# CityU-AIM-Group/HTD

Hardware: AMD Instinct MI355X
Metric: images/sec (1333x800) HTD-R50 train step (higher is better)
Workload: dtype f32; 1 GPU; HTD ResNet-50 FPN fp32 train step fwd+bwd+SGD, batch 4/GPU @ 1333x800 (padded 1344x800), random-init weights, 2000 RPN proposals/img, 512 RoIs/img/stage; global_batch=4, parallelism=dp1, stage2_positives=168, proposals=random-init RPN (few positives: the regression branch is nearly idle)

## Files before the change

### htd_amd/csrc/conv_x3.hip

```cpp
#include <algorithm>
#include <mutex>
#include <type_traits>
#include <unordered_map>

#include <stdlib.h>

#include "common.h"

namespace {

using f32x16 = __attribute__((ext_vector_type(16))) float;
using bf16x8 = __attribute__((ext_vector_type(8))) __bf16;
using bf16x2 = __attribute__((ext_vector_type(2))) __bf16;
using f32x2 = __attribute__((ext_vector_type(2))) float;
using f32x4 = __attribute__((ext_vector_type(4))) float;

using f16x8 = __attribute__((ext_vector_type(8))) _Float16;
using f16x2 = __attribute__((ext_vector_type(2))) _Float16;

constexpr int XK = 16;
constexpr int NCH = 6;

struct H2Scale { float s, inv; };
__device__ __forceinline__ H2Scale h2_scale(const float *amax)
// ... 1227 lines not shown
    int lo = 0, hi = n - 1;
    const int64_t b = blockIdx.x;
    while (lo < hi) {
        const int mid = (lo + hi + 1) >> 1;
        if (descs[mid].row0 <= b) lo = mid;
        else hi = mid - 1;
    }
    const PlanesDescH d = descs[lo];
    const int tr = d.transposed & 1;
    const int N = tr ? d.Ci : d.Co, K = tr ? d.Co : d.Ci;
    const int Np = ((N + 127) / 128) * 128;
    float *scales = reinterpret_cast<float *>(d.out + planes_vec(d.taps, K, Np));
    const int groups = Np / 64, r = (int)(b - d.row0);
    x3h_rowmax_part(d.w, scales + 2 * Np, d.Co, d.taps, d.Ci, Np, tr, (r % groups) * 64, r / groups, red);
}

__global__ __launch_bounds__(256) void x3h_planes_many_kernel(const PlanesDescH *__restrict__ descs, int n)
{
    int lo = 0, hi = n - 1;
    const int64_t b = blockIdx.x;
    while (lo < hi) {
        const int mid = (lo + hi + 1) >> 1;
        if (descs[mid].block0 <= b) lo = mid;
        else hi = mid - 1;
    }
    const PlanesDescH d = descs[lo];
    const int tr = d.transposed & 1;
    const int N = tr ? d.Ci : d.Co, K = tr ? d.Co : d.Ci;
    const int Np = ((N + 127) / 128) * 128;
    const int64_t total = (int64_t)d.taps * (K / XK) * Np;
    const int64_t e = (b - d.block0) * 256 + threadIdx.x;
    float *scales = reinterpret_cast<float *>(d.out + planes_vec(d.taps, K, Np));
    if (e < total) x3h_planes_element(d.w, d.out, scales, d.Co, d.taps, d.Ci, Np, tr, e);
}

__global__ __launch_bounds__(256) void absmax_kernel(const float *__restrict__ x, int64_t n, unsigned *__restrict__ out)
{
    const int64_t n4 = n >> 2;
    float mx = 0.f;
    unsigned nan = 0u;
    const float4 *x4 = reinterpret_cast<const float4 *>(x);
    const int64_t stride = (int64_t)gridDim.x * 256;
    int64_t i = (int64_t)blockIdx.x * 256 + threadIdx.x;
    for (; i + 3 * stride < n4; i += 4 * stride) {
        const float4 a = x4[i], b = x4[i + stride], c = x4[i + 2 * stride], d = x4[i + 3 * stride];
        const float m0 = fmaxf(fmaxf(fabsf(a.x), fabsf(a.y)), fmaxf(fabsf(a.z), fabsf(a.w)));
        const float m1 = fmaxf(fmaxf(fabsf(b.x), fabsf(b.y)), fmaxf(fabsf(b.z), fabsf(b.w)));
        const float m2 = fmaxf(fmaxf(fabsf(c.x), fabsf(c.y)), fmaxf(fabsf(c.z), fabsf(c.w)));
        const float m3 = fmaxf(fmaxf(fabsf(d.x), fabsf(d.y)), fmaxf(fabsf(d.z), fabsf(d.w)));
        mx = fmaxf(fmaxf(mx, fmaxf(m0, m1)), fmaxf(m2, m3));
        const float t = (a.x - a.x) + (a.y - a.y) + (a.z - a.z) + (a.w - a.w) + (b.x - b.x) + (b.y - b.y) + (b.z - b.z) + (b.w - b.w) +
                        (c.x - c.x) + (c.y - c.y) + (c.z - c.z) + (c.w - c.w) + (d.x - d.x) + (d.y - d.y) + (d.z - d.z) + (d.w - d.w);
        if (t != t) {
            nan |= (a.x != a.x) | (a.y != a.y) | (a.z != a.z) | (a.w != a.w) | (b.x != b.x) | (b.y != b.y) | (b.z != b.z) | (b.w != b.w) |
                   (c.x != c.x) | (c.y != c.y) | (c.z != c.z) | (c.w != c.w) | (d.x != d.x) | (d.y != d.y) | (d.z != d.z) | (d.w != d.w);
        }
    }
    for (; i < n4; i += stride) {
        const float4 v = x4[i];
        mx = fmaxf(fmaxf(mx, fmaxf(fabsf(v.x), fabsf(v.y))), fmaxf(fabsf(v.z), fabsf(v.w)));
        nan |= (v.x != v.x) | (v.y != v.y) | (v.z != v.z) | (v.w != v.w);
    }
    if (blockIdx.x == 0 && threadIdx.x < (n & 3)) {
        const float t = x[(n4 << 2) + threadIdx.x];
        mx = fmaxf(mx, fabsf(t));
        nan |= t != t;
// ... 378 lines not shown
                       Ci, Np, transposed);
    return htd::check_launch("x3h_planes");
}

extern "C" int htd_conv2d_x3h_planes_many(const void *desc, int n, int64_t total_blocks, int64_t total_rows, void *stream)
{
    static_assert(sizeof(PlanesDescH) == 48, "PlanesDescH layout is part of the ABI");
    HTD_REQUIRE(desc && n > 0 && total_blocks > 0 && total_blocks < (1ll << 31) && total_rows > 0 && total_rows < (1ll << 31),
                "x3h_planes_many: bad arguments");
    hipLaunchKernelGGL(x3h_rowscale_many_kernel, dim3((unsigned)total_rows), dim3(256), 0, (hipStream_t)stream,
                       (const PlanesDescH *)desc, n);
    hipLaunchKernelGGL(x3h_planes_many_kernel, dim3((unsigned)total_blocks), dim3(256), 0, (hipStream_t)stream,
                       (const PlanesDescH *)desc, n);
    return htd::check_launch("x3h_planes_many");
}

extern "C" int htd_absmax(const float *x, int64_t n, float *amax, void *stream)
{
    HTD_REQUIRE(x && amax && n > 0 && ((uintptr_t)x & 15) == 0, "absmax: bad arguments");
    const unsigned blocks = (unsigned)std::min<int64_t>(htd::ceil_div(n >> 2, (int64_t)256 * 8) + 1, 2048);
    hipLaunchKernelGGL(absmax_kernel, dim3(blocks), dim3(256), 0, (hipStream_t)stream, x, n, (unsigned *)amax);
    return htd::check_launch("absmax");
}

extern "C" int htd_conv2d_x3_planes_many(const void *desc, int n, int64_t total_blocks, void *stream)
{
    static_assert(sizeof(PlanesDesc) == 40, "PlanesDesc layout is part of the ABI");
    HTD_REQUIRE(desc && n > 0 && total_blocks > 0 && total_blocks < (1ll << 31), "x3_planes_many: bad arguments");
    hipLaunchKernelGGL(x3_planes_many_kernel, dim3((unsigned)total_blocks), dim3(256), 0, (hipStream_t)stream,
                       (const PlanesDesc *)desc, n);
    return htd::check_launch("x3_planes_many");
}

extern "C" int64_t htd_conv2d_x3p_workspace_bytes(int64_t M, int Co, int Ci, int kh, int kw)
{
    int64_t need = 0;
    for (int cfg = 0; cfg < 4; ++cfg) need = std::max(need, plan_x3p(cfg, M, Co, (Ci / XK) * kh, kw, true).partial_floats * 4);
    return need;
}

extern "C" int64_t htd_act_planes_rows(int64_t M) { return M > 0 ? act_rows(M) : 0; }

extern "C" int64_t htd_act_planes_bytes(int64_t M, int C)
{
    if (M <= 0 || C <= 0 || C % XK != 0) return 0;
    return (int64_t)(C / XK) * NCH * act_rows(M) * 16;
}

extern "C" int htd_act_planes(const float *x, void *planes, int64_t M, int C, void *stream)
{
    HTD_REQUIRE(x && planes && M > 0 && C > 0 && C % XK == 0, "act_planes: bad arguments (C %% 16)");
    const unsigned blocks = (unsigned)std::min<int64_t>(htd::ceil_div(M * (C >> 3), (int64_t)256), 65536);
    hipLaunchKernelGGL(act_planes_kernel, dim3(blocks), dim3(256), 0, (hipStream_t)stream, x, (uint4 *)planes, M, C, act_rows(M));
    return htd::check_launch("act_planes");
}

extern "C" int htd_conv2d_fwd_x3q(const float *x, const void *xplanes, const void *wplanes, const float *bias,
                                  const float *residual, int res_h, int res_w, float *y, void *yplanes, float *amax_out, int B, int H,
                                  int W, int Ci, int Co, int kh, int kw, int stride, int pad, int relu, void *workspace, void *stream)
{
    HTD_REQUIRE((x || xplanes) && wplanes && y && B > 0 && H > 0 && W > 0, "conv2d_fwd_x3q: bad arguments");
    HTD_REQUIRE(x3p_shape_ok(Ci, Co, kh, kw, stride, pad, 1), "conv2d_fwd_x3q: unsupported layer Ci=%d Co=%d k=%dx%d s=%d p=%d", Ci,
                Co, kh, kw, stride, pad);
    HTD_REQUIRE(!xplanes || (kh == 1 && stride == 1), "conv2d_fwd_x3q: input planes serve 1x1 / stride-1 layers only");
    HTD_REQUIRE(!yplanes || Co % XK == 0, "conv2d_fwd_x3q: output planes need Co %% 16 == 0 (Co=%d)", Co);
    HTD_REQUIRE((res_h > 0) == (res_w > 0) && res_h >= 0 && (res_h == 0 || ((Co & 3) == 0 && residual)),
// ... 214 lines not shown
```

### htd_amd/dense.py

```python
import os

import torch
from torch.autograd import Function
from torch.autograd.function import once_differentiable
from torch.multiprocessing.reductions import StorageWeakRef as _StorageWeakRef

from . import capi

CL = torch.channels_last
_P = capi.ptr
_S = capi.current_stream_ptr


def _out_hw(H, W, kh, kw, stride, pad, dil):
    return ((H + 2 * pad - (dil * (kh - 1) + 1)) // stride + 1, (W + 2 * pad - (dil * (kw - 1) + 1)) // stride + 1)


def _need_gpu(t, name):
    if not t.is_cuda:
        raise NotImplementedError(f'{name}: only GPU tensors are supported (libhtd_amd.so has no CPU path)')


def _splitk_ws(M, Co, Cred, kh, kw, device):
    nbytes = capi.lib().htd_conv2d_workspace_bytes(M, Co, Cred, kh, kw)
    return torch.empty(nbytes // 4, device=device, dtype=torch.float32) if nbytes > 0 else None


_GRAD_SINK = {}


def register_grad_sinks(params, views, used):
    import weakref
    keys = []
    for p, v in zip(params, views):
        _GRAD_SINK[p.data_ptr()] = (v, weakref.ref(p), used)
        keys.append(p.data_ptr())
    used.clear()
    return keys


# ... 112 lines not shown
    return s


def mark_side_consumed(t):
    _SIDE_CONSUMED.add(t.data_ptr())


_FLIPPED = {}


def offer_flipped(weight, wT):
    _FLIPPED[weight.data_ptr()] = wT


def take_flipped(weight):
    return _FLIPPED.pop(weight.data_ptr(), None)


_STEP_FLIPS = {}


_M = None


def _flip_key(w):
    global _M
    if _M is None:
        from . import mmcv_ops
        _M = mmcv_ops
    return (w.data_ptr(), w._version, tuple(w.shape), _M.PARAM_EPOCH)


def new_step():
    _STEP_FLIPS.clear()
    _STEP_PLANES.clear()
    _AMAX_POOL.clear()
    _AMAX_BY_PTR.clear()
    _drop_temp_sinks()


_AMAX_POOL = {}
_AMAX_SLOTS = 1024
H2_1X1 = os.environ.get('HTD_H2_1X1', '1') != '0'
H2_CHECK = os.environ.get('HTD_H2_CHECK', '0') == '1'
H2_ABSMAX_MIN_WORK = int(os.environ.get('HTD_H2_ABSMAX_MIN_WORK', '2304'))
H2_ABSMAX_MIN_ELEMS = int(os.environ.get('HTD_H2_ABSMAX_MIN_ELEMS', str(1 << 20)))


def _x3h_ok(Cred, Cout, kh, kw, stride, padding, dilation, dtype):
    return dtype == torch.float32 and (kh == 3 or H2_1X1) and \
        bool(capi.lib().htd_conv2d_x3h_supported(Cred, Cout, kh, kw, stride, padding, dilation))


def _amax_slot(device):
    ent = _AMAX_POOL.get(device.index)
    if ent is None or ent[1] >= _AMAX_SLOTS:
        ent = [torch.zeros(_AMAX_SLOTS, device=device, dtype=torch.float32), 0]
        _AMAX_POOL[device.index] = ent
    slot = ent[0][ent[1]:ent[1] + 1]
    ent[1] += 1
    return slot


def absmax(x):
    slot = _amax_slot(x.device)
    capi.call('htd_absmax', _P(x), x.numel(), _P(slot), _S(), work=('byte', 4.0 * x.numel()))
# ... 73 lines not shown
    if a is None or a[1] != t.data_ptr() or a[2] != t.numel() or a[3] != t._version:
        return None
    if H2_CHECK:
        fresh = absmax(t)
        if not torch.equal(fresh, a[0]) and not (torch.isnan(fresh).item() and torch.isnan(a[0]).item()):
            raise RuntimeError(f'stale carried maximum: {float(a[0])} against {float(fresh)} on a tensor of shape {tuple(t.shape)}')
    return a[0]


_STEP_PLANES = {}


def _planes_key(w, transposed):
    return _flip_key(w) + (bool(transposed), )


_ALSO_WANTED = set()


def _planes_h2(w, transposed):
    Co, Ci, kh, kw = w.shape
    cred, cout = (Co, Ci) if transposed else (Ci, Co)
    return kh == kw and _x3h_ok(cred, cout, kh, kw, 1, kh // 2, 1, w.dtype)


def x3_planes(weight, transposed, h2=None):
    if h2 is None:
        h2 = _planes_h2(weight, transposed)
    key = _planes_key(weight, transposed) + (bool(h2), )
    hit = _STEP_PLANES.get(key)
    if hit is not None:
        return hit[1]
    _ALSO_WANTED.add((tuple(weight.shape), bool(transposed), bool(h2)))
    Co, Ci, kh, kw = weight.shape
    nbytes = capi.lib().htd_conv2d_x3_planes_bytes(Co, kh, kw, Ci, int(transposed))
    planes = torch.empty(nbytes // 4, device=weight.device, dtype=torch.int32)
    capi.call('htd_conv2d_x3h_planes' if h2 else 'htd_conv2d_x3_planes', _P(weight), _P(planes), Co, kh, kw, Ci, int(transposed), _S())
    _STEP_PLANES[key] = (weight, planes)
    return planes


def _planes_wanted(w, transposed):
    Co, Ci, kh, kw = w.shape
    cred, cout = (Co, Ci) if transposed else (Ci, Co)
    return w.is_cuda and w.dtype == torch.float32 and kh == kw and kh in (1, 3) and w.is_contiguous(memory_format=CL) and \
        bool(capi.lib().htd_conv2d_x3p_supported(cred, cout, kh, kw, 1, kh // 2, 1))


def planes_many(items):
    import numpy as np
    todo, seen = [], set()
    for w, tr in items:
        w4 = w if w.dim() == 4 else w.view(w.size(0), w.size(1), 1, 1)
        if not _planes_wanted(w4, tr):
            continue
        h2 = _planes_h2(w4, tr)
        for v in ((h2, ) if (tuple(w4.shape), bool(tr), not h2) not in _ALSO_WANTED else (h2, not h2)):
            key = _planes_key(w4, tr) + (v, )
            if key not in _STEP_PLANES and key not in seen:
                seen.add(key)
                todo.append((key, w4, tr))
    if not todo:
        return
    L = capi.lib()
    dev = todo[0][1].device
    for h2 in (False, True):
# ... 4 lines not shown
        flat = torch.empty(sum(sizes), device=dev, dtype=torch.int32)
        desc = np.zeros((len(part), 6 if h2 else 5), dtype=np.int64)
        off = block0 = row0 = 0
        for i, ((key, w, tr), n32) in enumerate(zip(part, sizes)):
            out = flat[off:off + n32]
            off += n32
            Co, Ci, taps = w.size(0), w.size(1), w.size(2) * w.size(3)
            N = Ci if tr else Co
            Np = (N + 127) // 128 * 128
            desc[i, 0], desc[i, 1] = w.data_ptr(), out.data_ptr()
            desc[i, 2] = Co | (taps << 32)
            desc[i, 3] = Ci | (int(tr) << 32)
            desc[i, 4] = block0
            K = Co if tr else Ci
            nch = (taps * K + 1023) // 1024
            if h2:
                desc[i, 5] = row0
                row0 += Np // 64 * nch
            block0 += ((n32 - (2 + nch) * Np) // 4 // 6 + 255) // 256
            _STEP_PLANES[key] = (w, out)
        table = capi.upload_table(desc, dev)
        if h2:
            capi.call('htd_conv2d_x3h_planes_many', _P(table), len(part), block0, row0, _S())
        else:
            capi.call('htd_conv2d_x3_planes_many', _P(table), len(part), block0, _S())


def _x3p_ok(Cred, Cout, kh, kw, stride, padding, dilation, dtype):
    return dtype == torch.float32 and bool(capi.lib().htd_conv2d_x3p_supported(Cred, Cout, kh, kw, stride, padding, dilation))


def flip_many(weights):
    import numpy as np
    ws, pl = [], []
    for w in weights:
        w4 = w if w.dim() == 4 else w.view(w.size(0), w.size(1), 1, 1)
        pl += [(w4, False), (w4, True)]
        if w4.is_cuda and w4.dtype == torch.float32 and w4.size(0) % 8 == 0 and w4.is_contiguous(memory_format=CL) and \
                _flip_key(w4) not in _STEP_FLIPS and not _planes_wanted(w4, True):
            ws.append(w4)
    planes_many(pl)
    if not ws:
        return
    dev = ws[0].device
    flat = torch.empty(sum(w.numel() for w in ws), device=dev, dtype=torch.float32)
    desc = np.zeros((len(ws), 10), dtype=np.int64)
    off = tile0 = 0
    for i, w in enumerate(ws):
        Co, Ci, taps = w.size(0), w.size(1), w.size(2) * w.size(3)
        wT = flat[off:off + w.numel()]
        off += w.numel()
        desc[i, 0], desc[i, 7] = w.data_ptr(), wT.data_ptr()
        desc[i, 8] = Co | (Ci << 32)
        desc[i, 9] = taps | (tile0 << 32)
        tile0 += taps * ((Co + 31) // 32) * ((Ci + 31) // 32)
        _STEP_FLIPS[_flip_key(w)] = (w, wT)
    table = capi.upload_table(desc, dev)
    capi.call('htd_bn_fold_many_fwd', _P(table), len(ws), tile0, 0.0, _S())


def join_side_stream():
    if _SIDE:
        cur = torch.cuda.current_stream()
        s = _SIDE.get(cur.device.index)
        if s is not None:
            cur.wait_stream(s)
# ... 1069 lines not shown
```

### htd_amd/detector/bricks.py

```python
import torch
import torch.nn as nn
import torch.nn.functional as F

from .. import mmcv_ops as M
from ..registry import CONV_LAYERS

CL = torch.channels_last


def dense_conv2d(x, weight, bias=None, stride=1, padding=0, dilation=1, relu=False, residual=None, residual_up=False,
                 chain=False):
    from .. import dense
    if x.dtype == torch.bfloat16:
        y = dense.conv2d_bf16_autograd(x, weight, bias, stride, padding, dilation, relu, residual, residual_up)
        return (y, x) if chain else y
    return dense.conv2d(x, weight, bias, stride, padding, dilation, relu, residual, residual_up, chain)


@CONV_LAYERS.register_module('Conv')
@CONV_LAYERS.register_module('Conv2d')
class Conv2d(nn.Conv2d):

    def __init__(self, *args, **kwargs):
        super().__init__(*args, **kwargs)
# ... 72 lines not shown
        w, gamma, mean, var = ctx.saved_tensors
        Co = w.size(0)
        K = w.numel() // Co
        gwf = gwf.contiguous(memory_format=CL)
        gbf = gbf.contiguous()
        from .. import dense

        def launch():
            (gw, s1), (gg, s2), (gb, s3) = dense.grad_out2(w), dense.grad_out2(gamma), dense.grad_out2(ctx.beta_ref)
            capi.call('htd_bn_fold_bwd', capi.ptr(w), capi.ptr(gamma), capi.ptr(mean), capi.ptr(var), ctx.eps,
                      capi.ptr(gwf), capi.ptr(gbf), capi.ptr(gw), capi.ptr(gg), capi.ptr(gb), Co, K,
                      capi.current_stream_ptr())
            return (gw, gg, gb), s1 and s2 and s3
        if not dense.OVERLAP_WGRAD or (capi.profiling() and not dense._OVERLAP_IN_PROFILE):
            return launch()[0] + (None, None, None)
        main, side = torch.cuda.current_stream(), dense.side_stream(gwf.device)
        side.wait_stream(main)
        gwf.record_stream(side)
        gbf.record_stream(side)
        with torch.cuda.stream(side):
            outs, all_sinks = launch()
        if not all_sinks:
            for t in outs:
                t.record_stream(main)
            main.wait_stream(side)
        return outs + (None, None, None)


class _BNFoldMany(torch.autograd.Function):

    @staticmethod
    def forward(ctx, eps, want_flips, want_planes, *tensors):
        import numpy as np
        from .. import capi, dense
        n = len(tensors) // 5
        dev = tensors[0].device
        ws = [tensors[5 * i].contiguous(memory_format=CL) for i in range(n)]
        sizes = [(w.size(0), w.size(1), w.size(2) * w.size(3)) for w in ws]
        total = sum(2 * w.numel() + w.size(0) for w in ws) if want_flips else sum(w.numel() + w.size(0) for w in ws)
        flat = torch.empty(total, device=dev, dtype=torch.float32)
        desc = np.zeros((n, 10), dtype=np.int64)
        outs, flips, off, tile0 = [], [], 0, 0
        for i, (w, (Co, Ci, taps)) in enumerate(zip(ws, sizes)):
            wf = flat[off:off + w.numel()].view(Co, w.size(2), w.size(3), Ci).permute(0, 3, 1, 2)
            off += w.numel()
            bf = flat[off:off + Co]
            off += Co
            wT = None
            if want_flips:
                wT = flat[off:off + w.numel()]
                off += w.numel()
            g, b, m, v = tensors[5 * i + 1:5 * i + 5]
            desc[i, :8] = (w.data_ptr(), g.data_ptr(), b.data_ptr(), m.data_ptr(), v.data_ptr(), wf.data_ptr(), bf.data_ptr(),
                           wT.data_ptr() if wT is not None else 0)
            desc[i, 8] = Co | (Ci << 32)
            desc[i, 9] = taps | (tile0 << 32)
            tile0 += taps * ((Co + 31) // 32) * ((Ci + 31) // 32)
            outs += [wf, bf]
            flips.append(wT)
        table = capi.upload_table(desc, dev)
        capi.call('htd_bn_fold_many_fwd', capi.ptr(table), n, tile0, float(eps), capi.current_stream_ptr())
        if want_planes:
            dense.planes_many([(wf, False) for wf in outs[0::2]] + ([(wf, True) for wf in outs[0::2]] if want_flips else []))
        for wf, wT in zip(outs[0::2], flips):
            dense.mark_side_consumed(wf)
            if wT is not None:
                dense.offer_flipped(wf, wT)
        ctx.save_for_backward(*[t for i in range(n) for t in (ws[i], tensors[5 * i + 1], tensors[5 * i + 3], tensors[5 * i + 4])])
        ctx.beta_refs = [tensors[5 * i + 2] for i in range(n)]
        ctx.eps, ctx.n = float(eps), n
        return tuple(outs)

    @staticmethod
    @torch.autograd.function.once_differentiable
    def backward(ctx, *grads):
        import numpy as np
        from .. import capi, dense
        n, saved = ctx.n, ctx.saved_tensors
        dev = saved[0].device

        def launch():
            desc = np.zeros((n, 11), dtype=np.int64)
            outs, row0, all_sinks, keep = [], 0, True, []
            for i in range(n):
                w, gamma, mean, var = saved[4 * i:4 * i + 4]
                Co, K = w.size(0), w.numel() // w.size(0)
                gwf, gbf = grads[2 * i], grads[2 * i + 1]
                gwf = torch.zeros_like(w, memory_format=CL) if gwf is None else gwf.contiguous(memory_format=CL)
                gbf = torch.zeros(Co, device=dev) if gbf is None else gbf.contiguous()
                keep += [gwf, gbf]
                (gw, s1), (gg, s2), (gb, s3) = dense.grad_out2(w), dense.grad_out2(gamma), dense.grad_out2(ctx.beta_refs[i])
                all_sinks = all_sinks and s1 and s2 and s3
                desc[i, :9] = (w.data_ptr(), gamma.data_ptr(), mean.data_ptr(), var.data_ptr(), gwf.data_ptr(), gbf.data_ptr(),
                               gw.data_ptr(), gg.data_ptr(), gb.data_ptr())
                desc[i, 9] = Co | (K << 32)
                desc[i, 10] = row0
                row0 += Co
                outs.append((gw, gg, gb))
            table = capi.upload_table(desc, dev)
            capi.call('htd_bn_fold_many_bwd', capi.ptr(table), n, row0, ctx.eps, capi.current_stream_ptr())
            return outs, all_sinks, keep
        if not dense.OVERLAP_WGRAD or (capi.profiling() and not dense._OVERLAP_IN_PROFILE):
            outs = launch()[0]
        else:
            main, side = torch.cuda.current_stream(), dense.side_stream(dev)
            side.wait_stream(main)
            with torch.cuda.stream(side):
                outs, all_sinks, keep = launch()
            for t in keep:
                t.record_stream(side)
            if not all_sinks:
                for trio in outs:
                    for t in trio:
                        t.record_stream(main)
                main.wait_stream(side)
        res = [None, None, None]
        for gw, gg, gb in outs:
            res += [gw, gg, gb, None, None]
        return tuple(res)


def frozen_bn_fold_many(pairs, want_flips=True, want_planes=True):
    ok = torch.is_grad_enabled() and all(w.is_cuda and w.dtype == torch.float32 and (w.numel() // w.size(0)) % 4 == 0 and
                                          not bn.training for w, bn in pairs)
    if not ok or len({bn.eps for _, bn in pairs}) != 1:
        out = []
        for w, bn in pairs:
            out += frozen_bn_fold(w, bn)
        return out
    args = []
    for w, bn in pairs:
        args += [w, bn.weight, bn.bias, bn.running_mean, bn.running_var]
    return list(_BNFoldMany.apply(pairs[0][1].eps, bool(want_flips), bool(want_planes), *args))


def frozen_bn_fold(conv_weight, bn):
    if conv_weight.is_cuda and (conv_weight.numel() // conv_weight.size(0)) % 4 == 0:
        if torch.is_grad_enabled():
            return _BNFold.apply(conv_weight, bn.weight, bn.bias, bn.running_mean, bn.running_var, bn.eps)
        key = (M.PARAM_EPOCH, conv_weight.data_ptr(), conv_weight._version, bn.weight._version, bn.bias._version,
               bn.running_mean._version, bn.running_var._version)
        cached = bn.__dict__.get('_htd_fold_cache')
        if cached is None or cached[0] != key:
            cached = (key, _BNFold.apply(conv_weight, bn.weight, bn.bias, bn.running_mean, bn.running_var, bn.eps))
            bn.__dict__['_htd_fold_cache'] = cached
        return cached[1]
    s = bn.weight * torch.rsqrt(bn.running_var + bn.eps)
    return conv_weight * s.view(-1, 1, 1, 1), bn.bias - bn.running_mean * s


def kaiming_init(module, a=0, mode='fan_out', nonlinearity='relu', bias=0, distribution='normal'):
    if distribution == 'uniform':
        nn.init.kaiming_uniform_(module.weight, a=a, mode=mode, nonlinearity=nonlinearity)
    else:
        nn.init.kaiming_normal_(module.weight, a=a, mode=mode, nonlinearity=nonlinearity)
    if getattr(module, 'bias', None) is not None:
        nn.init.constant_(module.bias, bias)


def xavier_init(module, gain=1, bias=0, distribution='normal'):
    if distribution == 'uniform' and gain == 1 and hasattr(module, 'tile_shape'):
        module.xavier_uniform_()
# ... 67 lines not shown
```

### htd_amd/detector/resnet.py

```python
import math
import os

import torch
import torch.nn as nn
from torch.nn.modules.batchnorm import _BatchNorm

from .. import mmcv_ops as M
from ..dense import ResStageBf16Function, ResStageFunction
from ..registry import BACKBONES
from .bricks import build_conv_layer, build_norm_layer, constant_init, frozen_bn_fold, frozen_bn_fold_many, kaiming_init

CL = torch.channels_last
FUSE_BF16_STAGE = os.environ.get('HTD_BF16_STAGE', '1') != '0'


def conv_bn(conv, bn, x, relu=False, residual=None):
    if bn.training:
        y = bn(conv(x))
        if residual is not None:
            y = y + residual
        return torch.relu(y) if relu else y
    w, b = frozen_bn_fold(conv.weight, bn)
    return conv(x, relu=relu, residual=residual, weight=w, bias=b)

# ... 72 lines not shown

class ResLayer(nn.Sequential):
    def __init__(self, block, inplanes, planes, num_blocks, stride=1, avg_down=False, conv_cfg=None,
                 norm_cfg=dict(type='BN'), downsample_first=True, **kwargs):
        assert not avg_down and downsample_first, 'ResNetV1d / hourglass variants are outside the HTD path'
        self.block = block
        downsample = None
        if stride != 1 or inplanes != planes * block.expansion:
            downsample = nn.Sequential(
                build_conv_layer(conv_cfg, inplanes, planes * block.expansion, kernel_size=1, stride=stride, bias=False),
                build_norm_layer(norm_cfg, planes * block.expansion)[1])
        layers = [block(inplanes=inplanes, planes=planes, stride=stride, downsample=downsample, conv_cfg=conv_cfg,
                        norm_cfg=norm_cfg, **kwargs)]
        inplanes = planes * block.expansion
        for _ in range(1, num_blocks):
            layers.append(block(inplanes=inplanes, planes=planes, stride=1, conv_cfg=conv_cfg, norm_cfg=norm_cfg,
                                **kwargs))
        super().__init__(*layers)

    def _fusable(self):
        for blk in self:
            if not isinstance(blk, Bottleneck) or blk.with_dcn or blk.style != 'pytorch' or blk.groups != 1:
                return False
            bns = [blk.norm1, blk.norm2, blk.norm3] + ([blk.downsample[1]] if blk.downsample is not None else [])
            if any(bn.training or not isinstance(bn, nn.BatchNorm2d) for bn in bns):
                return False
        return True

    def forward(self, x, chain=False):
        if not x.is_cuda or x.dtype not in (torch.float32, torch.bfloat16) or not self._fusable() or \
                (x.dtype == torch.bfloat16 and not FUSE_BF16_STAGE):
            y = super().forward(x)
            return (y, x) if chain else y
        pairs = []
        for blk in self:
            pairs += [(blk.conv1.weight, blk.norm1), (blk.conv2.weight, blk.norm2), (blk.conv3.weight, blk.norm3)]
            if blk.downsample is not None:
                pairs.append((blk.downsample[0].weight, blk.downsample[1]))
        params = frozen_bn_fold_many(pairs, want_flips=x.dtype == torch.float32 and
                                     (x.requires_grad or any(w.requires_grad for w, _ in pairs)),
                                     want_planes=x.dtype == torch.float32)
        strides, has_ds = tuple(blk.conv2_stride for blk in self), tuple(blk.downsample is not None for blk in self)
        if x.dtype == torch.float32:
            use = bool(chain and x.requires_grad and torch.is_grad_enabled() and strides[0] == 1)
            y = ResStageFunction.apply(x, strides, self[0].dilation, has_ds, use, *params)
            if chain:
                return y if use else (y, x)
            return y
        y = ResStageBf16Function.apply(x, strides, self[0].dilation, has_ds, *params)
        return (y, x) if chain else y


@BACKBONES.register_module()
class ResNet(nn.Module):
    arch_settings = {50: (Bottleneck, (3, 4, 6, 3)), 101: (Bottleneck, (3, 4, 23, 3)), 152: (Bottleneck, (3, 8, 36, 3))}

    def __init__(self, depth, in_channels=3, stem_channels=None, base_channels=64, num_stages=4,
                 strides=(1, 2, 2, 2), dilations=(1, 1, 1, 1), out_indices=(0, 1, 2, 3), style='pytorch',
                 deep_stem=False, avg_down=False, frozen_stages=-1, conv_cfg=None,
                 norm_cfg=dict(type='BN', requires_grad=True), norm_eval=True, dcn=None,
                 stage_with_dcn=(False, False, False, False), plugins=None, with_cp=False, zero_init_residual=True):
        super().__init__()
        if depth not in self.arch_settings:
            raise KeyError(f'invalid depth {depth} for resnet')
        assert not deep_stem and not avg_down and plugins is None
        self.depth = depth
        stem_channels = base_channels if stem_channels is None else stem_channels
        self.stem_channels, self.base_channels, self.num_stages = stem_channels, base_channels, num_stages
        assert 1 <= num_stages <= 4
        self.strides, self.dilations = strides, dilations
        assert len(strides) == len(dilations) == num_stages
        self.out_indices = out_indices
        assert max(out_indices) < num_stages
        self.style, self.deep_stem, self.avg_down, self.frozen_stages = style, deep_stem, avg_down, frozen_stages
# ... 109 lines not shown
```

### htd_amd/mmcv_ops.py

```python
import ctypes
import os

import torch
import torch.nn as nn
from torch.autograd import Function
from torch.autograd.function import once_differentiable

from . import capi

CL = torch.channels_last


def _drop_amax(t):
    from . import dense
    dense.drop_amax(t)


def _need_gpu(t, name):
    if not t.is_cuda:
        raise NotImplementedError(f'{name}: only GPU tensors are supported (libhtd_amd.so has no CPU path)')


def nhwc(x):
    return x.contiguous(memory_format=CL)
# ... 707 lines not shown
        ctx.meta = (int(num_groups), int(bool(relu)))
        ctx.bias_ref = bias
        return y

    @staticmethod
    @once_differentiable
    def backward(ctx, gy):
        x, y, weight, mean, rstd = ctx.saved_tensors
        G, relu = ctx.meta
        n, C, h, w = x.shape
        gy = nhwc(gy)
        gx = torch.empty_like(x, memory_format=CL)
        from . import dense
        gw = dense.grad_out(weight)
        gb = dense.grad_out(ctx.bias_ref) if ctx.bias_ref is not None and ctx.bias_ref.shape == weight.shape else torch.empty_like(weight)
        ws = torch.empty(2 * max(n, 1) * C, device=x.device, dtype=torch.float32)
        L = capi.lib()
        if n > 0 and L.htd_conv2d_set_h2(-1) == 1 and L.htd_group_norm_bwd_amax_supported(h * w, C, G):
            slot = dense._amax_slot(x.device)
            capi.call('htd_group_norm_relu_bwd_amax', _P(x), _P(y), _P(weight), _P(mean), _P(rstd), _P(gy), _P(gx), _P(gw),
                      _P(gb), n, h * w, C, G, relu, _P(ws), _P(slot), _S(), key='htd_group_norm_relu_bwd_ws')
            dense.tag_amax(gx, slot)
        else:
            capi.call('htd_group_norm_relu_bwd_ws', _P(x), _P(y), _P(weight), _P(mean), _P(rstd), _P(gy), _P(gx), _P(gw),
                      _P(gb), n, h * w, C, G, relu, _P(ws), _S())
        return gx, gw, gb, None, None, None


def group_norm_relu(x, weight, bias, num_groups, eps=1e-5, relu=True):
    return GroupNormReLUFunction.apply(x, weight, bias, num_groups, eps, relu)


PARAM_EPOCH = 0


def sgd_momentum_step_(flat_param, flat_grad, flat_momentum, lr_dev, momentum, weight_decay, grad_scale=1.0):
    _need_gpu(flat_param, 'sgd')
    global PARAM_EPOCH
    PARAM_EPOCH += 1
    capi.call('htd_sgd_momentum_step', _P(flat_param), _P(flat_grad), _P(flat_momentum), flat_param.numel(),
              _P(lr_dev), float(momentum), float(weight_decay), float(grad_scale), _S())


def log_accumulator(n, device):
    acc = torch.zeros(n + 2, dtype=torch.float64, device=device)
    acc[n + 1] = -1.0
    return acc


def log_accumulate_(acc, packed, weight, it, loss_index=-1):
    n = packed.numel()
    loss_index = loss_index % n
    if acc.dtype != torch.float64 or acc.numel() != n + 2 or packed.dtype != torch.float32 or not packed.is_contiguous():
        raise ValueError(f'log_accumulate: acc must be fp64 [{n + 2}] and packed contiguous fp32, got {acc.dtype} '
                         f'[{acc.numel()}] / {packed.dtype}')
    if packed.is_cuda:
        capi.call('htd_log_accumulate', _P(packed), n, loss_index, float(weight), int(it), _P(acc), _S())
        return acc
    acc[:n] += packed.double() * float(weight)
    acc[n] += float(weight)
    if float(acc[n + 1]) < 0 and not bool(torch.isfinite(packed[loss_index])):
        acc[n + 1] = float(it)
    return acc


TOPK_CHUNK, TOPK_KMAX = 4096, 2048
_TOPK_PLANS = {}


def segmented_topk(keys, segments):
    _need_gpu(keys, 'segmented_topk')
    keys = _f32(keys, 'segmented_topk')
# ... 205 lines not shown
```

### include/htd_amd.h

```cpp
#ifndef HTD_AMD_H
#define HTD_AMD_H

#include <stdint.h>

#ifdef __cplusplus
extern "C" {
#endif

#define HTD_OK 0
#define HTD_ERR_ARG 1
#define HTD_ERR_LAUNCH 2

const char *htd_last_error(void);
#define HTD_ABI_VERSION 7
int htd_abi_version(void);

int htd_roi_align_fwd(const float *feat, const float *rois, const int64_t *roi_level, int level,
                      float *out, int64_t n, int B, int C, int H, int W, int ph, int pw, float spatial_scale,
                      int sampling_ratio, int aligned, void *stream);
int htd_roi_align_bwd(const float *grad_out, const float *rois, const int64_t *roi_level, int level,
                      float *grad_feat, int64_t n, int B, int C, int H, int W, int ph, int pw,
                      float spatial_scale, int sampling_ratio, int aligned, void *stream);
int htd_roi_align_levels_fwd(const float *const *feats, const int *H, const int *W, const float *scales, int L,
                             const float *rois, const int64_t *roi_level, float *out, int64_t n, int B, int C, int ph, int pw,
// ... 111 lines not shown
int htd_conv2d_x3_planes_many(const void *desc, int n, int64_t total_blocks, void *stream);
int64_t htd_conv2d_x3p_workspace_bytes(int64_t M, int Co, int Ci, int kh, int kw);
int htd_conv2d_fwd_x3p(const float *x, const void *wplanes, const float *bias, const float *residual, int res_h,
                       int res_w, float *y, int B, int H, int W, int Ci, int Co, int kh, int kw, int stride, int pad,
                       int relu, void *workspace, void *stream);
int htd_conv2d_bwd_data_x3p(const float *gy, const void *wplanesT, const float *mask_src, const float *accum,
                            float *gx, int B, int H, int W, int Ci, int Co, int kh, int kw, int pad, void *workspace,
                            void *stream);
int64_t htd_act_planes_rows(int64_t M);
int64_t htd_act_planes_bytes(int64_t M, int C);
int htd_act_planes(const float *x, void *planes, int64_t M, int C, void *stream);
int htd_conv2d_fwd_x3q(const float *x, const void *xplanes, const void *wplanes, const float *bias, const float *residual,
                       int res_h, int res_w, float *y, void *yplanes, float *amax_out, int B, int H, int W, int Ci, int Co, int kh, int kw,
                       int stride, int pad, int relu, void *workspace, void *stream);
int htd_conv2d_bwd_data_x3q(const float *gy, const void *gyplanes, const void *wplanesT, const float *mask_src,
                            const float *accum, float *gx, void *gxplanes, float *amax_out, int B, int H, int W, int Ci, int Co, int kh, int kw,
                            int pad, void *workspace, void *stream);

int htd_conv2d_set_h2(int on);
int htd_conv2d_bwd_weight_h2_supported(int B, int H, int W, int Ci, int Co, int kh, int kw, int stride, int pad, int dil);
int htd_conv2d_bwd_weight_h2(const float *x, const float *gy, const float *amax_x, const float *amax_g, float *gw,
                             float *gbias, int B, int H, int W, int Ci, int Co, int kh, int kw, int stride, int pad,
                             int dil, int accumulate, void *workspace, void *stream);
int htd_conv2d_x3h_supported(int Ci, int Co, int kh, int kw, int stride, int pad, int dil);
int htd_conv2d_x3h_strided_supported(int Ci, int Co, int kh, int kw, int stride, int pad, int dil);
int htd_conv2d_bwd_data_x3h_strided_supported(int Ci, int Co, int kh, int kw, int stride, int pad, int dil);
int64_t htd_conv2d_bwd_data_x3h_strided_workspace_bytes(int B, int H, int W, int Ci, int Co, int kh, int kw, int stride, int pad);
int htd_conv2d_bwd_data_x3h_strided(const float *gy, const float *amax, const void *wplanesT, const float *mask_src, float *gx,
                                    float *amax_out, int B, int H, int W, int Ci, int Co, int kh, int kw, int stride, int pad,
                                    void *workspace, void *stream);
int htd_absmax(const float *x, int64_t n, float *amax, void *stream);
int htd_conv2d_x3h_planes(const float *w, void *planes, int Co, int kh, int kw, int Ci, int transposed, void *stream);
int htd_conv2d_x3h_planes_many(const void *desc, int n, int64_t total_blocks, int64_t total_rows, void *stream);
int htd_conv2d_fwd_x3h(const float *x, const float *amax, const void *wplanes, const float *bias, const float *residual,
                       int res_h, int res_w, float *y, void *yplanes, float *amax_out, int B, int H, int W, int Ci,
                       int Co, int kh, int kw, int stride, int pad, int relu, void *workspace, void *stream);
int htd_conv2d_bwd_data_x3h(const float *gy, const float *amax, const void *wplanesT, const float *mask_src,
                            const float *accum, float *gx, void *gxplanes, float *amax_out, int B, int H, int W,
                            int Ci, int Co, int kh, int kw, int pad, void *workspace, void *stream);

int64_t htd_deform_columns_bytes(int B, int H, int W, int C, int kh, int kw, int stride, int pad, int dil);
int htd_deform_im2col(const float *x, const float *offset, const float *mask, float *columns, int B,
                      int H, int W, int C, int kh, int kw, int stride, int pad, int dil,
                      int deform_groups, void *stream);
int htd_deform_col2im(const float *x, const float *offset, const float *mask, const float *gcolumns,
                      float *gx, float *goffset, float *gmask, int B, int H, int W, int C, int kh,
                      int kw, int stride, int pad, int dil, int deform_groups, void *stream);
int htd_deform_im2col_bf16(const void *x, const float *offset, const float *mask, void *columns, int B, int H, int W,
                           int C, int kh, int kw, int stride, int pad, int dil, int deform_groups, void *stream);
int htd_deform_col2im_bf16(const void *x, const float *offset, const float *mask, const void *gcolumns, float *gx,
                           float *goffset, float *gmask, int B, int H, int W, int C, int kh, int kw, int stride, int pad,
                           int dil, int deform_groups, void *stream);

int htd_global_avg_pool_fwd(const float *x, float *out, int64_t B, int P, int C, void *stream);
int htd_global_avg_pool_bwd(const float *g, float *gx, int64_t B, int P, int C, void *stream);
int htd_global_avg_pool_bwd_acc(const float *g, float *gx, int64_t B, int P, int C, void *stream);

int htd_group_norm_relu_fwd(const float *x, const float *gamma, const float *beta, float *y,
                            float *mean, float *rstd, int64_t n, int P, int C, int G, float eps,
                            int relu, void *stream);
int htd_group_norm_relu_bwd(const float *x, const float *y, const float *gamma, const float *mean,
                            const float *rstd, const float *gy, float *gx, float *ggamma,
                            float *gbeta, int64_t n, int P, int C, int G, int relu, void *stream);
int htd_group_norm_relu_bwd_ws(const float *x, const float *y, const float *gamma, const float *mean, const float *rstd,
                               const float *gy, float *gx, float *ggamma, float *gbeta, int64_t n, int P, int C, int G,
                               int relu, void *workspace, void *stream);
// ... 169 lines not shown
```

Baseline: 120.4 images/sec.

## Batch per-step weight preparation into one cached multi-kernel arena launch

Adds a registry of conv weights with their frozen-BN parameters. Each step, all weight preparation for that registry runs in one batched launch: BN folding, transposed/flipped copies, per-chunk absmax scales and x3/x3h plane images, all written into a single arena. Results are keyed on tensor pointers and versions plus the optimizer epoch, so frozen-stage weights are reused across steps and only trainable ones are rebuilt. The aim is to remove many small per-layer kernel launches and host-side table uploads, at the cost of more Python bookkeeping and a risk of serving stale images if invalidation misses a change.

```diff
diff --git a/htd_amd/csrc/conv_x3.hip b/htd_amd/csrc/conv_x3.hip
--- a/htd_amd/csrc/conv_x3.hip
+++ b/htd_amd/csrc/conv_x3.hip
@@ -1283,6 +1283,137 @@
     const int64_t e = (b - d.block0) * 256 + threadIdx.x;
     float *scales = reinterpret_cast<float *>(d.out + planes_vec(d.taps, K, Np));
     if (e < total) x3h_planes_element(d.w, d.out, scales, d.Co, d.taps, d.Ci, Np, tr, e);
+}
+
+struct PrepDesc {
+    const float *w, *gamma, *beta, *mean, *var;
+    int64_t wf, bf, wT;
+    int64_t img[4];
+    int Co, Ci, taps, tile0;
+    int64_t block0;
+    float eps;
+    int pad;
+};
+
+__device__ __forceinline__ int prep_find(const PrepDesc *__restrict__ d, int n, int64_t idx, bool tiles)
+{
+    int lo = 0, hi = n - 1;
+    while (lo < hi) {
+        const int mid = (lo + hi + 1) >> 1;
+        if ((tiles ? (int64_t)d[mid].tile0 : d[mid].block0) <= idx) lo = mid; else hi = mid - 1;
+    }
+    return lo;
+}
+
+__device__ __forceinline__ float *prep_parts(char *arena, int64_t img, int taps, int N, int K)
+{
+    const int Np = ((N + 127) / 128) * 128;
+    return reinterpret_cast<float *>(reinterpret_cast<uint4 *>(arena + img) + planes_vec(taps, K, Np)) + 2 * Np;
+}
+
+__global__ __launch_bounds__(256) void weight_prep_zero_kernel(const PrepDesc *__restrict__ descs, char *__restrict__ arena)
+{
+    const PrepDesc d = descs[blockIdx.x >> 1];
+    const int tr = blockIdx.x & 1;
+    const int64_t img = d.img[2 * tr + 1];
+    if (img < 0) return;
+    const int N = tr ? d.Ci : d.Co, K = tr ? d.Co : d.Ci;
+    const int Np = ((N + 127) / 128) * 128;
+    float *part = prep_parts(arena, img, d.taps, N, K);
+    const int total = h2_chunks(d.taps, K) * Np;
+    for (int i = threadIdx.x; i < total; i += 256) part[i] = 0.f;
+}
+
+__global__ __launch_bounds__(256) void weight_prep_fold_kernel(const PrepDesc *__restrict__ descs, int n, char *__restrict__ arena)
+{
+    __shared__ float tile[32][33];
+    const PrepDesc d = descs[prep_find(descs, n, blockIdx.x, true)];
+    const int nco = (d.Co + 31) / 32, nci = (d.Ci + 31) / 32;
+    int idx = (int)blockIdx.x - d.tile0;
+    const int ci_t = idx % nci;
+    idx /= nci;
+    const int co_t = idx % nco, t = idx / nco;
+    const int co0 = co_t * 32, ci0 = ci_t * 32;
+    const int tx = threadIdx.x & 31, ty = threadIdx.x >> 5;
+    float *wf = d.wf >= 0 ? reinterpret_cast<float *>(arena + d.wf) : nullptr;
+    for (int r = ty; r < 32; r += 8) {
+        const int co = co0 + r, ci = ci0 + tx;
+        float v = 0.f;
+        if (co < d.Co && ci < d.Ci) {
+            const int64_t i = ((int64_t)co * d.taps + t) * d.Ci + ci;
+            if (d.gamma) {
+                v = d.w[i] * (d.gamma[co] * rsqrtf(d.var[co] + d.eps));
+                wf[i] = v;
+            } else
+                v = d.w[i];
+        }
+        tile[r][tx] = v;
+    }
+    if (d.gamma && t == 0 && ci_t == 0 && ty == 0 && co0 + tx < d.Co) {
+        const int co = co0 + tx;
+        const float s = d.gamma[co] * rsqrtf(d.var[co] + d.eps);
+        reinterpret_cast<float *>(arena + d.bf)[co] = d.beta[co] - d.mean[co] * s;
+    }
+    const bool h2f = d.img[1] >= 0, h2t = d.img[3] >= 0;
+    if (d.wT < 0 && !h2f && !h2t) return;
+    __syncthreads();
+    if (d.wT >= 0) {
+        float *wT = reinterpret_cast<float *>(arena + d.wT);
+        for (int r = ty; r < 32; r += 8) {
+            const int ci = ci0 + r, co = co0 + tx;
+            if (ci < d.Ci && co < d.Co) wT[((int64_t)ci * d.taps + (d.taps - 1 - t)) * d.Co + co] = tile[tx][r];
+        }
+    }
+    if (threadIdx.x < 64) {
+        const bool col = threadIdx.x >= 32;
+        if (col ? !h2t : !h2f) return;
+        const int n_ = col ? ci0 + tx : co0 + tx, N = col ? d.Ci : d.Co, K = col ? d.Co : d.Ci;
+        if (n_ >= N) return;
+        const int e_first = col ? co0 * d.taps + t : t * d.Ci + ci0, e_step = col ? d.taps : 1;
+        const int kmax = min(32, (col ? d.Co - co0 : d.Ci - ci0));
+        const int Np = ((N + 127) / 128) * 128;
+        unsigned *part = reinterpret_cast<unsigned *>(prep_parts(arena, d.img[col ? 3 : 1], d.taps, N, K)) + n_;
+        float m = 0.f;
+        int c = e_first / H2_ECH;
+        for (int k = 0; k < kmax; ++k) {
+            const int ck = (e_first + k * e_step) / H2_ECH;
+            if (ck != c) {
+                if (m > 0.f) atomicMax(part + (int64_t)c * Np, __float_as_uint(m));
+                m = 0.f;
+                c = ck;
+            }
+            m = fmaxf(m, fabsf(col ? tile[k][tx] : tile[tx][k]));
+        }
+        if (m > 0.f) atomicMax(part + (int64_t)c * Np, __float_as_uint(m));
+    }
+}
+
+__global__ __launch_bounds__(256) void weight_prep_planes_kernel(const PrepDesc *__restrict__ descs, int n, char *__restrict__ arena)
+{
+    const PrepDesc d = descs[prep_find(descs, n, blockIdx.x, false)];
+    int64_t b = (int64_t)blockIdx.x - d.block0;
+    const float *src = d.gamma ? reinterpret_cast<const float *>(arena + d.wf) : d.w;
+#pragma unroll
+    for (int v = 0; v < 4; ++v) {
+        if (d.img[v] < 0) continue;
+        const int tr = v >> 1;
+        const int N = tr ? d.Ci : d.Co, K = tr ? d.Co : d.Ci;
+        const int Np = ((N + 127) / 128) * 128;
+        const int64_t total = (int64_t)d.taps * (K / XK) * Np, blocks = (total + 255) / 256;
+        if (b >= blocks) {
+            b -= blocks;
+            continue;
+        }
+        const int64_t e = b * 256 + threadIdx.x;
+        uint4 *out = reinterpret_cast<uint4 *>(arena + d.img[v]);
+        if (e < total) {
+            if (v & 1)
+                x3h_planes_element(src, out, reinterpret_cast<float *>(out + planes_vec(d.taps, K, Np)), d.Co, d.taps, d.Ci, Np, tr, e);
+            else
+                x3_planes_element(src, out, d.Co, d.taps, d.Ci, Np, tr, e);
+        }
+        return;
+    }
 }
 
 __global__ __launch_bounds__(256) void absmax_kernel(const float *__restrict__ x, int64_t n, unsigned *__restrict__ out)
@@ -1727,6 +1858,23 @@
     return htd::check_launch("x3_planes_many");
 }
 
+extern "C" int htd_weight_prep_many(const void *desc, int n, int64_t total_tiles, int64_t total_blocks, void *arena, void *stream)
+{
+    static_assert(sizeof(PrepDesc) == 128, "PrepDesc layout is part of the ABI");
+    HTD_REQUIRE(desc && arena && n > 0 && n < (1 << 30) && total_tiles >= 0 && total_tiles < (1ll << 31) && total_blocks >= 0 &&
+                total_blocks < (1ll << 31) && ((uintptr_t)arena & 15) == 0, "weight_prep_many: bad arguments");
+    const PrepDesc *d = (const PrepDesc *)desc;
+    if (total_tiles > 0) {
+        hipLaunchKernelGGL(weight_prep_zero_kernel, dim3(2u * (unsigned)n), dim3(256), 0, (hipStream_t)stream, d, (char *)arena);
+        hipLaunchKernelGGL(weight_prep_fold_kernel, dim3((unsigned)total_tiles), dim3(256), 0, (hipStream_t)stream, d, n,
+                           (char *)arena);
+    }
+    if (total_blocks > 0)
+        hipLaunchKernelGGL(weight_prep_planes_kernel, dim3((unsigned)total_blocks), dim3(256), 0, (hipStream_t)stream, d, n,
+                           (char *)arena);
+    return htd::check_launch("weight_prep_many");
+}
+
 extern "C" int64_t htd_conv2d_x3p_workspace_bytes(int64_t M, int Co, int Ci, int kh, int kw)
 {
     int64_t need = 0;
diff --git a/htd_amd/dense.py b/htd_amd/dense.py
--- a/htd_amd/dense.py
+++ b/htd_amd/dense.py
@@ -5,7 +5,7 @@
 from torch.autograd.function import once_differentiable
 from torch.multiprocessing.reductions import StorageWeakRef as _StorageWeakRef
 
-from . import capi
+from . import capi, weight_prep
 
 CL = torch.channels_last
 _P = capi.ptr
@@ -184,6 +184,7 @@
 
 
 def new_step():
+    weight_prep.new_step()
     _STEP_FLIPS.clear()
     _STEP_PLANES.clear()
     _AMAX_POOL.clear()
@@ -323,6 +324,7 @@
     if hit is not None:
         return hit[1]
     _ALSO_WANTED.add((tuple(weight.shape), bool(transposed), bool(h2)))
+    weight_prep.note_single(weight, transposed, h2)
     Co, Ci, kh, kw = weight.shape
     nbytes = capi.lib().htd_conv2d_x3_planes_bytes(Co, kh, kw, Ci, int(transposed))
     planes = torch.empty(nbytes // 4, device=weight.device, dtype=torch.int32)
@@ -393,6 +395,8 @@
 
 def flip_many(weights):
     import numpy as np
+    if weight_prep.plain_lookup(weights):
+        return
     ws, pl = [], []
     for w in weights:
         w4 = w if w.dim() == 4 else w.view(w.size(0), w.size(1), 1, 1)
diff --git a/htd_amd/detector/bricks.py b/htd_amd/detector/bricks.py
--- a/htd_amd/detector/bricks.py
+++ b/htd_amd/detector/bricks.py
@@ -128,10 +128,14 @@
     @staticmethod
     def forward(ctx, eps, want_flips, want_planes, *tensors):
         import numpy as np
-        from .. import capi, dense
+        from .. import capi, dense, weight_prep
         n = len(tensors) // 5
         dev = tensors[0].device
         ws = [tensors[5 * i].contiguous(memory_format=CL) for i in range(n)]
+        hit = weight_prep.fold_lookup(tensors, n, float(eps), want_flips, want_planes)
+        if hit is not None:
+            outs, flips = hit
+            return _BNFoldMany._finish(ctx, eps, n, ws, tensors, outs, flips)
         sizes = [(w.size(0), w.size(1), w.size(2) * w.size(3)) for w in ws]
         total = sum(2 * w.numel() + w.size(0) for w in ws) if want_flips else sum(w.numel() + w.size(0) for w in ws)
         flat = torch.empty(total, device=dev, dtype=torch.float32)
@@ -158,6 +162,11 @@
         capi.call('htd_bn_fold_many_fwd', capi.ptr(table), n, tile0, float(eps), capi.current_stream_ptr())
         if want_planes:
             dense.planes_many([(wf, False) for wf in outs[0::2]] + ([(wf, True) for wf in outs[0::2]] if want_flips else []))
+        return _BNFoldMany._finish(ctx, eps, n, ws, tensors, outs, flips)
+
+    @staticmethod
+    def _finish(ctx, eps, n, ws, tensors, outs, flips):
+        from .. import dense
         for wf, wT in zip(outs[0::2], flips):
             dense.mark_side_consumed(wf)
             if wT is not None:
@@ -216,7 +225,7 @@
         return tuple(res)
 
 
-def frozen_bn_fold_many(pairs, want_flips=True, want_planes=True):
+def frozen_bn_fold_many(pairs, want_flips=True, want_planes=True, keep_flips=()):
     ok = torch.is_grad_enabled() and all(w.is_cuda and w.dtype == torch.float32 and (w.numel() // w.size(0)) % 4 == 0 and
                                           not bn.training for w, bn in pairs)
     if not ok or len({bn.eps for _, bn in pairs}) != 1:
@@ -224,6 +233,8 @@
         for w, bn in pairs:
             out += frozen_bn_fold(w, bn)
         return out
+    from .. import weight_prep
+    weight_prep.note_fold(pairs, pairs[0][1].eps, want_flips, want_planes, keep_flips)
     args = []
     for w, bn in pairs:
         args += [w, bn.weight, bn.bias, bn.running_mean, bn.running_var]
diff --git a/htd_amd/detector/resnet.py b/htd_amd/detector/resnet.py
--- a/htd_amd/detector/resnet.py
+++ b/htd_amd/detector/resnet.py
@@ -128,14 +128,16 @@
                 (x.dtype == torch.bfloat16 and not FUSE_BF16_STAGE):
             y = super().forward(x)
             return (y, x) if chain else y
-        pairs = []
+        pairs, strided = [], []
         for blk in self:
+            if blk.conv2_stride != 1:
+                strided += [len(pairs) + 1] + ([len(pairs) + 3] if blk.downsample is not None else [])
             pairs += [(blk.conv1.weight, blk.norm1), (blk.conv2.weight, blk.norm2), (blk.conv3.weight, blk.norm3)]
             if blk.downsample is not None:
                 pairs.append((blk.downsample[0].weight, blk.downsample[1]))
         params = frozen_bn_fold_many(pairs, want_flips=x.dtype == torch.float32 and
                                      (x.requires_grad or any(w.requires_grad for w, _ in pairs)),
-                                     want_planes=x.dtype == torch.float32)
+                                     want_planes=x.dtype == torch.float32, keep_flips=tuple(strided))
         strides, has_ds = tuple(blk.conv2_stride for blk in self), tuple(blk.downsample is not None for blk in self)
         if x.dtype == torch.float32:
             use = bool(chain and x.requires_grad and torch.is_grad_enabled() and strides[0] == 1)
diff --git a/htd_amd/mmcv_ops.py b/htd_amd/mmcv_ops.py
--- a/htd_amd/mmcv_ops.py
+++ b/htd_amd/mmcv_ops.py
@@ -763,12 +763,14 @@
 
 
 PARAM_EPOCH = 0
+OPT_STEPS = 0
 
 
 def sgd_momentum_step_(flat_param, flat_grad, flat_momentum, lr_dev, momentum, weight_decay, grad_scale=1.0):
     _need_gpu(flat_param, 'sgd')
-    global PARAM_EPOCH
+    global PARAM_EPOCH, OPT_STEPS
     PARAM_EPOCH += 1
+    OPT_STEPS += 1
     capi.call('htd_sgd_momentum_step', _P(flat_param), _P(flat_grad), _P(flat_momentum), flat_param.numel(),
               _P(lr_dev), float(momentum), float(weight_decay), float(grad_scale), _S())
 
diff --git a/htd_amd/weight_prep.py b/htd_amd/weight_prep.py
--- /dev/null
+++ b/htd_amd/weight_prep.py
@@ -0,0 +1,286 @@
+import os
+import weakref
+
+import numpy as np
+import torch
+
+from . import capi
+
+ENABLED = os.environ.get('HTD_WEIGHT_PREP', '1') != '0'
+CALLS = 0
+CL = torch.channels_last
+_P, _S = capi.ptr, capi.current_stream_ptr
+
+_REG = {}
+_GEN = 0
+_STEP = 0
+
+
+class _Entry:
+    __slots__ = ('ref', 'shape', 'bn', 'eps', 'flips', 'planes', 'keep', 'frozen', 'kinds', 'born', 'key', 'seg', 'out')
+
+    def weight(self):
+        w = self.ref()
+        if w is None or tuple(w.shape) == self.shape:
+            return w
+        Co, Ci, kh, kw = self.shape
+        return w.as_strided(self.shape, (Ci * kh * kw, 1, kw * Ci, Ci))
+
+    def bn_tensors(self):
+        bn = self.bn() if self.bn is not None else None
+        return None if bn is None else (bn.weight, bn.bias, bn.running_mean, bn.running_var)
+
+    def state(self):
+        w = self.ref()
+        if w is None:
+            return None
+        k = (w.data_ptr(), w._version)
+        if self.bn is not None:
+            ts = self.bn_tensors()
+            if ts is None:
+                return None
+            for t in ts:
+                k += (t.data_ptr(), t._version)
+        return k
+
+
+class _Set:
+    def __init__(self, frozen):
+        self.frozen = frozen
+        self.sig = self.checked = self.key = self.table = self.ptrs = self.arena = self.desc = None
+        self.entries, self.sizes, self.tiles, self.blocks = [], [], 0, 0
+
+
+_SETS = {False: _Set(False), True: _Set(True)}
+
+
+def new_step():
+    global _STEP
+    _STEP += 1
+
+
+def _shape4(w):
+    return tuple(w.shape) if w.dim() == 4 else (w.size(0), w.size(1), 1, 1)
+
+
+def _dense_weight(w):
+    return w.is_cuda and w.dtype == torch.float32 and \
+        (w.is_contiguous(memory_format=CL) if w.dim() == 4 else (w.dim() == 2 and w.is_contiguous()))
+
+
+def _register(w, shape, bn, eps, flips, planes, keep, kinds=None):
+    global _GEN
+    key = (w.data_ptr(), shape)
+    frozen = bn is not None and not (w.requires_grad or bn.weight.requires_grad or bn.bias.requires_grad)
+    e = _REG.get(key)
+    if e is not None and e.ref() is w and (bn is None if e.bn is None else e.bn() is bn) and \
+            (e.eps, e.flips, e.planes, e.keep, e.frozen) == (eps, flips, planes, keep, frozen):
+        if kinds is not None and not kinds <= e.kinds:
+            e.kinds |= kinds
+            _GEN += 1
+        return
+    e = _Entry()
+    e.ref, e.shape, e.bn = weakref.ref(w), shape, (None if bn is None else weakref.ref(bn))
+    e.eps, e.flips, e.planes, e.keep, e.frozen, e.kinds = eps, flips, planes, keep, frozen, kinds
+    e.key = e.seg = e.out = None
+    e.born = _STEP
+    _REG[key] = e
+    _GEN += 1
+
+
+def note_fold(pairs, eps, want_flips, want_planes, keep_flips=()):
+    if ENABLED:
+        for i, (w, bn) in enumerate(pairs):
+            if w.dim() == 4 and _dense_weight(w):
+                _register(w, tuple(w.shape), bn, float(eps), bool(want_flips), bool(want_planes), i in keep_flips)
+
+
+def note_single(weight, transposed, h2):
+    if not ENABLED or weight.dim() != 4 or not weight.is_contiguous(memory_format=CL):
+        return
+    shape = tuple(weight.shape)
+    own = _REG.get((weight.data_ptr(), shape))
+    if own is not None and own.kinds is None:
+        return
+    for (ptr, _), e in list(_REG.items()):
+        w = e.ref()
+        if ptr == weight.data_ptr() and e.bn is None and w is not None and w.numel() == weight.numel() and \
+                w.data_ptr() == ptr and w._version == weight._version:
+            _register(w, shape, None, 0.0, False, False, False, kinds={(bool(transposed), bool(h2))})
+            return
+
+
+def _layout(s):
+    from . import dense
+    L = capi.lib()
+    for e in s.entries:
+        e.seg = e.out = e.key = None
+    ents = []
+    for key, e in list(_REG.items()):
+        if e.ref() is None or (e.bn is not None and e.bn() is None) or e.ref().data_ptr() != key[0]:
+            del _REG[key]
+        elif e.frozen == s.frozen:
+            ents.append(e)
+    desc = np.zeros((len(ents), 16), dtype=np.int64)
+    sizes, tiles, blocks = [], 0, 0
+
+    def seg(nfloats):
+        sizes.append((nfloats + 3) // 4 * 4)
+        return len(sizes) - 1
+    for i, e in enumerate(ents):
+        w4 = e.weight()
+        Co, Ci, kh, kw = e.shape
+        taps = kh * kw
+        e.seg = dict(wf=None, bf=None, wT=None, img={})
+        if e.bn is not None:
+            e.seg['wf'], e.seg['bf'] = seg(w4.numel()), seg(Co)
+        if e.kinds is not None:
+            kinds = sorted(e.kinds)
+        else:
+            kinds = []
+            wanted_t = dense._planes_wanted(w4, True)
+            if e.flips and (e.keep or not wanted_t) and (e.bn is not None or Co % 8 == 0):
+                e.seg['wT'] = seg(w4.numel())
+            for tr in ((False, True) if e.flips else (False, )):
+                if e.planes and (wanted_t if tr else dense._planes_wanted(w4, False)):
+                    h2 = dense._planes_h2(w4, tr)
+                    kinds.append((tr, h2))
+                    if (e.shape, tr, not h2) in dense._ALSO_WANTED:
+                        kinds.append((tr, not h2))
+        kinds = [(tr, h2) for tr, h2 in kinds if (Co if tr else Ci) % 16 == 0 and (tr or Ci % 4 == 0)]
+        for tr, h2 in kinds:
+            e.seg['img'][(tr, h2)] = seg(L.htd_conv2d_x3_planes_bytes(Co, kh, kw, Ci, int(tr)) // 4)
+        desc[i, 5:12] = -1
+        desc[i, 12] = Co | (Ci << 32)
+        desc[i, 13] = taps | (tiles << 32)
+        desc[i, 14] = blocks
+        desc[i, 15] = int(np.float32(e.eps).view(np.uint32))
+        if e.bn is not None or e.seg['wT'] is not None or any(h2 for _, h2 in kinds):
+            tiles += taps * ((Co + 31) // 32) * ((Ci + 31) // 32)
+        for tr, _ in kinds:
+            N, K = (Ci, Co) if tr else (Co, Ci)
+            blocks += (taps * (K // 16) * ((N + 127) // 128 * 128) + 255) // 256
+    offs = np.concatenate([[0], np.cumsum(np.asarray(sizes, dtype=np.int64))]) * 4
+    for i, e in enumerate(ents):
+        for j, name in enumerate(('wf', 'bf', 'wT')):
+            if e.seg[name] is not None:
+                desc[i, 5 + j] = offs[e.seg[name]]
+        for (tr, h2), k in e.seg['img'].items():
+            desc[i, 8 + 2 * int(tr) + int(h2)] = offs[k]
+    s.entries, s.sizes, s.tiles, s.blocks, s.desc = ents, sizes, tiles, blocks, desc
+    s.table = s.ptrs = s.key = None
+
+
+def _validate(s):
+    from . import dense, mmcv_ops as M
+    global CALLS
+    token = (_STEP, M.PARAM_EPOCH)
+    if s.checked == token:
+        return bool(s.entries)
+    sig = (_GEN, len(dense._ALSO_WANTED))
+    if s.sig != sig or any(e.state() is None for e in s.entries):
+        _layout(s)
+        s.sig = sig
+    s.checked = token
+    if not s.entries or not s.sizes:
+        return False
+    states = tuple(e.state() for e in s.entries)
+    key = (M.PARAM_EPOCH - M.OPT_STEPS if s.frozen else M.PARAM_EPOCH, states)
+    if key == s.key:
+        return True
+    ptrs = tuple(st[0::2] for st in states)
+    dev = s.entries[0].ref().device
+    if s.table is None or s.ptrs != ptrs:
+        for i, row in enumerate(ptrs):
+            s.desc[i, :5] = 0
+            s.desc[i, :len(row)] = row
+        s.table, s.ptrs = capi.upload_table(s.desc, dev), ptrs
+    s.arena = torch.empty(sum(s.sizes), device=dev, dtype=torch.float32)
+    capi.call('htd_weight_prep_many', _P(s.table), len(s.entries), s.tiles, s.blocks, _P(s.arena), _S())
+    CALLS += 1
+    parts = s.arena.split(s.sizes)
+    for e, st in zip(s.entries, states):
+        Co, Ci, kh, kw = e.shape
+        n, o = Co * Ci * kh * kw, e.seg
+        e.key = st
+        e.out = dict(wf=None if o['wf'] is None else parts[o['wf']][:n].view(Co, kh, kw, Ci).permute(0, 3, 1, 2),
+                     bf=None if o['bf'] is None else parts[o['bf']][:Co],
+                     wT=None if o['wT'] is None else parts[o['wT']][:n],
+                     img={k: parts[v] for k, v in o['img'].items()})
+    s.key = key
+    return True
+
+
+def _ready(ents):
+    for again in (False, True):
+        for frozen in {e.frozen for e in ents}:
+            if not _validate(_SETS[frozen]):
+                return False
+        stale = [e for e in ents if e.out is None or e.key != e.state()]
+        if not stale:
+            return True
+        if again or any(e.out is None for e in stale):
+            return False
+        for e in stale:
+            _SETS[e.frozen].checked = None
+    return False
+
+
+def _offer_images(e, src):
+    from . import dense
+    base = dense._flip_key(src)
+    for (tr, h2), img in e.out['img'].items():
+        dense._STEP_PLANES[base + (tr, h2)] = (src, img)
+
+
+def fold_lookup(tensors, n, eps, want_flips, want_planes):
+    if not ENABLED:
+        return None
+    ents = []
+    for i in range(n):
+        w = tensors[5 * i]
+        e = _REG.get((w.data_ptr(), tuple(w.shape)))
+        ts = e.bn_tensors() if e is not None and e.bn is not None else None
+        if ts is None or e.ref() is None or (e.eps, e.flips, e.planes) != (eps, want_flips, want_planes) or \
+                e.born >= _STEP or any(a.data_ptr() != b.data_ptr() for a, b in zip(ts, tensors[5 * i + 1:5 * i + 5])):
+            return None
+        ents.append(e)
+    if not _ready(ents):
+        return None
+    outs, flips = [], []
+    for e in ents:
+        wf = e.out['wf'].detach()
+        _offer_images(e, wf)
+        outs += [wf, e.out['bf'].detach()]
+        flips.append(e.out['wT'])
+    return outs, flips
+
+
+def plain_lookup(weights):
+    if not ENABLED:
+        return False
+    from . import dense
+    ents, known = [], True
+    for w in weights:
+        if not _dense_weight(w):
+            continue
+        e = _REG.get((w.data_ptr(), _shape4(w)))
+        if e is None or e.ref() is not w or e.bn is not None or e.kinds is not None or e.born >= _STEP:
+            known = False
+            break
+        ents.append(e)
+    if not known:
+        for w in weights:
+            if _dense_weight(w):
+                _register(w, _shape4(w), None, 0.0, True, True, False)
+        return False
+    ptrs = {e.ref().data_ptr() for e in ents}
+    ents += [e for (ptr, _), e in _REG.items() if e.kinds is not None and ptr in ptrs and e.ref() is not None and e.born < _STEP]
+    if not ents or not _ready(ents):
+        return False
+    for e in ents:
+        w4 = e.weight()
+        _offer_images(e, w4)
+        if e.out['wT'] is not None:
+            dense._STEP_FLIPS[dense._flip_key(w4)] = (w4, e.out['wT'])
+    return True
diff --git a/include/htd_amd.h b/include/htd_amd.h
--- a/include/htd_amd.h
+++ b/include/htd_amd.h
@@ -167,6 +167,7 @@
 int htd_absmax(const float *x, int64_t n, float *amax, void *stream);
 int htd_conv2d_x3h_planes(const float *w, void *planes, int Co, int kh, int kw, int Ci, int transposed, void *stream);
 int htd_conv2d_x3h_planes_many(const void *desc, int n, int64_t total_blocks, int64_t total_rows, void *stream);
+int htd_weight_prep_many(const void *desc, int n, int64_t total_tiles, int64_t total_blocks, void *arena, void *stream);
 int htd_conv2d_fwd_x3h(const float *x, const float *amax, const void *wplanes, const float *bias, const float *residual,
                        int res_h, int res_w, float *y, void *yplanes, float *amax_out, int B, int H, int W, int Ci,
                        int Co, int kh, int kw, int stride, int pad, int relu, void *workspace, void *stream);
```

Result: slower. 99.50 images/sec (-17.4%).
